# antbern/gridmap-slam-robot

Hardware: AMD Instinct MI355X
Metric: particle-scan evals/sec (higher is better)
Workload: dtype f64; 1 GPU; C3: 16384 particles/GPU x 720 beams (697 hits), 2048x2048 grid @ 0.02 m, full scan step (score+normalise+resample+ray-cast+likelihood rebuild; the rebuild is dirty-tile / factor-table-only: bit-identical results, likelihoodData on demand -- the reference's own every-cell rebuild is cpu_baseline.gpu_like_for_like_ms_per_step); particles_total=16384, particles_per_gpu=16384, beams=720, maps=1, maps_total=1, parallelism=single GPU, inputs=resident in HBM

## Files before the change

### gridmap_slam_robot_amd/csrc/gms_device.h

```cpp
#pragma once

#include <hip/hip_runtime.h>
#include <stdint.h>

#include "gms_internal.h"

#define GMS_WAVE 64

__device__ __forceinline__ void store_through(double *p, double v) { __hip_atomic_store(p, v, __ATOMIC_RELAXED, __HIP_MEMORY_SCOPE_AGENT); }
__device__ __forceinline__ void store_through(uint64_t *p, uint64_t v) { __hip_atomic_store(p, v, __ATOMIC_RELAXED, __HIP_MEMORY_SCOPE_AGENT); }

#define GMS_STAMP_SLOTS 16
#ifdef GMS_STAMPS
__device__ unsigned long long *g_gms_stamps;
#define GMS_STAMP_T(tid, row, slot) do { if (g_gms_stamps && threadIdx.x == (tid)) g_gms_stamps[(size_t)(row) * GMS_STAMP_SLOTS + (slot)] = wall_clock64(); } while (0)
#else
#define GMS_STAMP_T(tid, row, slot) do { } while (0)
#endif
#define GMS_STAMP(row, slot) GMS_STAMP_T(0, row, slot)
#define GMS_STAMP_ROW(kernel_id, wg) ((kernel_id) * 1024u + ((wg) < 1023u ? (wg) : 1023u))

__device__ __forceinline__ int32_t j_d2i(double d) {
    if (d != d) return 0;
    if (d >= 2147483647.0) return INT32_MAX;
    if (d <= -2147483648.0) return INT32_MIN;
// ... 200 lines not shown
```

### gridmap_slam_robot_amd/csrc/gms_fused_kernels.hip

```cpp
#include "gms_map_kernels.hip"
#include "gms_pf_kernels.hip"
#include "gms_slam_kernels.hip"

#ifndef GMS_APPLY_BLOCKS_RIDING
#define GMS_APPLY_BLOCKS_RIDING 512
#endif

#ifndef RCF_RAYS
#define RCF_RAYS 4
#endif

template <bool LOGNORM>
__global__ void __launch_bounds__(256)
k_norm_raycast(GridDev g, const gms_beam *__restrict__ beams, int32_t B, uint32_t *__restrict__ cnt, int32_t *__restrict__ bbox,
               int32_t nw_max, uint32_t n_ray_blocks,
               const double *__restrict__ partials, int64_t nblk_global, double *__restrict__ w, const float *__restrict__ pose,
               int32_t n, int64_t offset, PackedParticle *__restrict__ packed, double *__restrict__ cum,
               double *__restrict__ chunk_tot, int64_t nchunks, double *__restrict__ p2, PfStatsDev *__restrict__ stats,
               uint32_t n_norm_blocks, double *__restrict__ logd, uint32_t *__restrict__ cnt_pend, const int32_t *__restrict__ bbox_pend,
               uint32_t n_near_blocks, const double *__restrict__ logw_lognorm) {
    extern __shared__ __align__(16) unsigned char smem[];
    GMS_STAMP(GMS_STAMP_ROW(2, blockIdx.x), 0);
    if (blockIdx.x >= n_ray_blocks + n_norm_blocks) {
        apply_body(g, logd, cnt_pend, bbox_pend, nullptr, blockIdx.x - n_ray_blocks - n_norm_blocks, 0,
                   gridDim.x - n_ray_blocks - n_norm_blocks);
        GMS_STAMP(GMS_STAMP_ROW(2, blockIdx.x), 15);
        return;
    }
    if (blockIdx.x < n_ray_blocks) {
        __shared__ RedLds L;
        __shared__ float s_pose[3];
        const int cols[4] = { COL_SUM, COL_XW, COL_YW, COL_TW };
        double f[4];
        if (LOGNORM) {
            fold_lognorm<4>(partials, nblk_global, cols, f, L);
// ... 2 lines not shown
        }
        if (threadIdx.x == 0) {
            s_pose[0] = (float)(f[1] / f[0]);
            s_pose[1] = (float)(f[2] / f[0]);
            s_pose[2] = (float)(f[3] / f[0]);
        }
        __syncthreads();
        GMS_STAMP(GMS_STAMP_ROW(2, blockIdx.x), 1);
        if (blockIdx.x >= n_ray_blocks - n_near_blocks)
            raycast_near_body(g, beams, B, B, nullptr, 0, cnt, bbox, blockIdx.x - (n_ray_blocks - n_near_blocks), 0, smem, s_pose);
        else
            raycast_body<false, RCF_RAYS, 4>(g, beams, B, B, nullptr, 0, nullptr, cnt, bbox, nullptr, nullptr, 0, nullptr, nw_max, blockIdx.x, 0,
                                             smem, s_pose, n_near_blocks ? 1 : 0);
    } else {
        normalize_pack_body(partials, nblk_global, w, pose, n, offset, packed, cum, chunk_tot, nchunks, p2, stats,
                            blockIdx.x - n_ray_blocks, 0, LOGNORM ? logw_lognorm : (const double *)nullptr);
        GMS_STAMP(GMS_STAMP_ROW(2, blockIdx.x), 14);
    }
}

__global__ void __launch_bounds__(256)
k_partials_apply(double *__restrict__ w, double *__restrict__ logw, const float *__restrict__ pose, int32_t n, int64_t offset,
                 int64_t nblk_global, double *__restrict__ partials, const double *__restrict__ part, int32_t part_nseg,
                 GridDev g, double *__restrict__ logd, uint32_t *__restrict__ cnt, const int32_t *__restrict__ bbox,
                 int32_t *__restrict__ bbox_idle, PfStatsDev *__restrict__ lognorm_stats) {
    if (blockIdx.x < (uint32_t)nblk_global)
        partials_body(w, logw, pose, n, offset, nblk_global, partials, part, part_nseg, blockIdx.x, blockIdx.y, lognorm_stats);
    else
        apply_body(g, logd, cnt, bbox, bbox_idle, blockIdx.x - (uint32_t)nblk_global, blockIdx.y, gridDim.x - (uint32_t)nblk_global);
}

// ... 48 lines not shown
        chunk_sums_raw_body(glob_raw, n_global, nchunks, cum, chunk_tot, p2, nblk_global, partials,
                            blockIdx.x - n_ray_blocks - n_norm_blocks);
    }
}

template <int KH, int SPLIT>
__global__ void __launch_bounds__(256)
k_lik_resample(GridDev g, const double *__restrict__ logd, double *__restrict__ lik, double *__restrict__ fac, int64_t fac_stride,
               const double *__restrict__ taps_g, const int32_t *__restrict__ bbox, int32_t tiles_x, int32_t tiles_y,
               const uint32_t *__restrict__ cnt_pending, uint8_t *__restrict__ tile_state, uint32_t n_res_blocks,
               const PackedParticle *__restrict__ glob, int64_t n_global, int64_t nchunks, const double *__restrict__ cum,
               const double *__restrict__ chunk_off, const double *__restrict__ r01_maps, double r01, double fraction,
               int32_t n, int64_t offset,
               float *__restrict__ pose2, float *__restrict__ cs2, double *__restrict__ w2, int32_t *__restrict__ idx_out,
               const double *__restrict__ p2, int64_t nblk_global, PfStatsDev *__restrict__ stats, int32_t raw_weights,
               int32_t *__restrict__ bbox_clear, int32_t lik_mode) {
    extern __shared__ __align__(16) unsigned char smem[];
    GMS_STAMP(GMS_STAMP_ROW(3, blockIdx.x), 0);
    if (blockIdx.x == 0 && threadIdx.x < 4) bbox_clear[4 * blockIdx.y + threadIdx.x] = 0;
    if (blockIdx.x < n_res_blocks)
        resample_body(glob, n_global, nchunks, cum, chunk_off, r01_maps, r01, fraction, n, offset, pose2, cs2, w2, idx_out, p2,
                      nblk_global, stats, blockIdx.x, blockIdx.y, smem, raw_weights != 0);
    else
        likelihood_body<KH, SPLIT>(g, logd, lik, fac, fac_stride, taps_g, bbox, 1, tiles_x, tiles_y, blockIdx.x - n_res_blocks,
                                   blockIdx.y, gridDim.x - n_res_blocks, smem, cnt_pending, tile_state, lik_mode);
    GMS_STAMP(GMS_STAMP_ROW(3, blockIdx.x), blockIdx.x < n_res_blocks ? 1 : 2);
}

__global__ void __launch_bounds__(256)
k_deskew_motion(const double *__restrict__ angle, const double *__restrict__ distance, const uint8_t *__restrict__ hit, int32_t length,
                double d_center, double d_theta, gms_beam *__restrict__ beams_out, uint32_t n_deskew_blocks,
                float *__restrict__ pose, float *__restrict__ cs, int32_t n, int64_t offset, double d_center_sd, double d_theta_sd,
                uint64_t seed, uint64_t sequence) {
    if (blockIdx.x < n_deskew_blocks)
        deskew_body(angle, distance, hit, length, d_center, d_theta, beams_out, (int32_t)(blockIdx.x * 256u + threadIdx.x));
    else
        motion_body(pose, cs, n, offset, d_center, d_theta, d_center_sd, d_theta_sd, seed, sequence, 0,
                    (int32_t)((blockIdx.x - n_deskew_blocks) * 256u + threadIdx.x));
}

bool gms_can_pair_launches(const gms_pf *pf, int32_t B) {
    const gms_map *m = pf->map;
    return pf->n_maps == 1 && B > 0 && B <= GMS_MAX_BEAMS && !m->need_full_build && m->pair_launches;
}

void gms_launch_norm_raycast(gms_pf *pf, const double *d_partials, PackedParticle *d_packed_local, bool own,
                             const gms_beam *d_beams, int32_t B) {
    gms_map *m = pf->map;
    ProfScope ps(m, GMS_K_RAYCAST);
    if (own) { pf->d_global = pf->d_global_own; pf->global_raw = 0; }
    const uint32_t n_near = rc_near_blocks(m, B);
    const uint32_t n_ray = (uint32_t)((B + RCF_RAYS - 1) / RCF_RAYS) + n_near, n_norm = (uint32_t)((pf->n + 255) / 256);
    const size_t smem = rc_smem(m, RCF_RAYS, n_near);
    uint32_t n_apply = 0;
    if (m->apply_pending) {
        const int32_t all = ((m->gd.W + APPLY_TW - 1) / APPLY_TW) * ((m->gd.H + APPLY_TH - 1) / APPLY_TH);
        n_apply = (uint32_t)(all < GMS_APPLY_BLOCKS_RIDING ? all : GMS_APPLY_BLOCKS_RIDING);
    }
    int32_t *pend = m->d_bbox + (size_t)m->bbox_cur * 4;
    int32_t *bb = n_apply ? m->d_bbox + (size_t)(1 - m->bbox_cur) * 4 : pend;
    const bool lognorm = gms_pf_lognorm_now(pf);
#define NR_LAUNCH(LN)                                                                                                                 \
    do {                                                                                                                              \
        if (smem > 48 * 1024)                                                                                                         \
            hipFuncSetAttribute(reinterpret_cast<const void *>(&k_norm_raycast<LN>), hipFuncAttributeMaxDynamicSharedMemorySize, (int)smem); \
        hipLaunchKernelGGL(k_norm_raycast<LN>, dim3(n_ray + n_norm + n_apply), dim3(256), smem, m->stream, m->gd, d_beams, B, m->d_cnt, bb, \
                           rc_nw_max(m), n_ray, d_partials, nblk_global_of(pf), pf->d_w, pf->d_pose, pf->n, pf->offset, d_packed_local, \
                           own ? pf->d_cum : (double *)nullptr, own ? pf->d_chunk_tot : (double *)nullptr, nchunks_of(pf),          \
                           own ? pf->d_p2 : (double *)nullptr, pf->d_stats, n_norm, m->d_log, m->d_cnt_pend, pend, n_near,          \
                           LN ? (const double *)pf->d_logw : (const double *)nullptr);                                              \
    } while (0)
    if (lognorm) NR_LAUNCH(true); else NR_LAUNCH(false);
#undef NR_LAUNCH
    pf->score_fresh = 0;
    if (n_apply) gms_apply_done(m);
    pf->chunks_ready = own ? 1 : 0;
    pf->neff_folded = 0;
}

void gms_launch_partials_apply(gms_pf *pf, double *d_partials, bool apply_rides_later) {
    gms_map *m = pf->map;
    if (!m->apply_pending || apply_rides_later) { gms_launch_pf_partials(pf, d_partials); return; }
    ProfScope ps(m, GMS_K_REDUCE);
    const int64_t nblk = nblk_global_of(pf);
    const int32_t all = ((m->gd.W + APPLY_TW - 1) / APPLY_TW) * ((m->gd.H + APPLY_TH - 1) / APPLY_TH);
    const uint32_t n_apply = (uint32_t)(all < GMS_APPLY_BLOCKS ? all : GMS_APPLY_BLOCKS);
    int32_t *cur = m->d_bbox + (size_t)m->bbox_cur * m->n_maps * 4, *idle = m->d_bbox + (size_t)(1 - m->bbox_cur) * m->n_maps * 4;
    PfStatsDev *lognorm_stats = gms_pf_lognorm_now(pf) ? pf->d_stats : (PfStatsDev *)nullptr;
    hipLaunchKernelGGL(k_partials_apply, dim3((uint32_t)nblk + n_apply, pf->n_maps), dim3(256), 0, m->stream, pf->d_w, pf->d_logw,
                       pf->d_pose, pf->n, pf->offset, nblk, d_partials,
                       pf->pending_nseg ? (const double *)pf->d_part : (const double *)nullptr, pf->pending_nseg, m->gd, m->d_log,
                       m->d_cnt_pend, cur, idle, lognorm_stats);
    pf->pending_nseg = 0;
    gms_apply_done(m);
}

void gms_launch_lik_resample(gms_pf *pf, double fraction) {
    gms_map *m = pf->map;
    gms_launch_pf_chunk_sums(pf);
    ProfScope ps(m, GMS_K_LIKELIHOOD);
    const int32_t k = m->lik_kh;
    const int32_t tiles_x = (m->gd.W + LK_TW - 1) / LK_TW, tiles_y = (m->gd.H + LK_TH - 1) / LK_TH;
    const size_t smem_l = gms_likelihood_lds_bytes(m->gd.khalf, k != 0);
    int32_t blocks = tiles_x * tiles_y;
    const int32_t cap = gms_likelihood_blocks_cap(m, smem_l);
    if (blocks > cap) blocks = cap;
    blocks = (blocks + 7) & ~7;
    const int64_t nch = nchunks_of(pf);
    const size_t smem_r = gms_resample_lds_bytes(nch);
    const size_t smem = smem_l > smem_r ? smem_l : smem_r;
    const uint32_t n_res = (uint32_t)((pf->n + 255) / 256);
    const int32_t *bb = m->d_bbox + (size_t)m->bbox_cur * m->n_maps * 4;
    const double *r01_maps = pf->n_maps == 1 ? (const double *)nullptr : pf->d_r01_src;
    int32_t lik_mode = m->lik_lazy ? 2 : 3;
    if (m->lik_lazy) m->lik_stale = 1;
    if (m->fac_current && m->lik_skip) lik_mode |= 4;
    m->fac_current = 1;
    const bool split = k != 0 && gms_likelihood_split(m, blocks);
#define LR_LAUNCH(KH, SP)                                                                                                 \
    do {                                                                                                                  \
        if (smem > 48 * 1024)                                                                                             \
            hipFuncSetAttribute(reinterpret_cast<const void *>(&k_lik_resample<KH, SP>),                                 \
                                hipFuncAttributeMaxDynamicSharedMemorySize, (int)smem);                                   \
        hipLaunchKernelGGL((k_lik_resample<KH, SP>), dim3((uint32_t)blocks + n_res, pf->n_maps), dim3(256), smem, m->stream, m->gd, m->d_log, \
                           m->d_lik, m->d_fac, m->fac_stride, m->d_taps, bb, tiles_x, tiles_y, m->d_cnt, m->d_tile_state, n_res, pf->d_global, \
                           pf->n_global, nch, pf->d_cum, pf->d_chunk_tot, r01_maps, pf->r01_scalar, fraction, pf->n, pf->offset, \
                           pf->d_pose2, pf->d_cs2, pf->d_w2, pf->d_idx, pf->d_p2, nblk_global_of(pf), pf->d_stats,       \
                           pf->global_raw, m->d_bbox + (size_t)(1 - m->bbox_cur) * m->n_maps * 4, lik_mode);             \
    } while (0)
    if (k == 3) { if (split) LR_LAUNCH(3, 2); else LR_LAUNCH(3, 1); }
    else if (k == 5) { if (split) LR_LAUNCH(5, 2); else LR_LAUNCH(5, 1); }
    else LR_LAUNCH(0, 1);
#undef LR_LAUNCH
    pf->neff_folded = 1;
}

void gms_launch_partials_pack_apply(gms_pf *pf, bool apply_rides_later) {
    gms_map *m = pf->map;
    ProfScope ps(m, GMS_K_REDUCE);
    const uint32_t n_local = (uint32_t)((pf->n + GMS_BLOCK - 1) / GMS_BLOCK);
    uint32_t n_apply = 0;
    if (m->apply_pending && !apply_rides_later) {
        const int32_t all = ((m->gd.W + APPLY_TW - 1) / APPLY_TW) * ((m->gd.H + APPLY_TH - 1) / APPLY_TH);
// ... 23 lines not shown
        const int32_t all = ((m->gd.W + APPLY_TW - 1) / APPLY_TW) * ((m->gd.H + APPLY_TH - 1) / APPLY_TH);
        n_apply = (uint32_t)(all < GMS_APPLY_BLOCKS_RIDING ? all : GMS_APPLY_BLOCKS_RIDING);
    }
    int32_t *pend = m->d_bbox + (size_t)m->bbox_cur * 4;
    int32_t *bb = n_apply ? m->d_bbox + (size_t)(1 - m->bbox_cur) * 4 : pend;
    if (smem > 48 * 1024)
        hipFuncSetAttribute(reinterpret_cast<const void *>(&k_raycast_norm_chunks), hipFuncAttributeMaxDynamicSharedMemorySize,
                            (int)smem);
    hipLaunchKernelGGL(k_raycast_norm_chunks, dim3(n_ray + n_norm + n_chunk + n_apply), dim3(256), smem, m->stream, m->gd, d_beams, B,
                       m->d_cnt, bb, rc_nw_max(m), n_ray, n_norm, pf->d_partials, nblk_global_of(pf), pf->d_w, pf->d_pose, pf->n,
                       pf->offset, pf->d_global_own, pf->n_global, nchunks_of(pf), pf->d_cum, pf->d_chunk_tot, pf->d_p2, pf->d_stats,
                       n_chunk, m->d_log, m->d_cnt_pend, pend, n_near);
    if (n_apply) gms_apply_done(m);
    pf->chunks_ready = 1;
    pf->neff_folded = 0;
}

void gms_launch_deskew_motion(gms_pf *pf, const double *d_angle, const double *d_distance, const uint8_t *d_hit, int32_t length,
                              double d_center, double d_theta, uint64_t seed, uint64_t sequence) {
    gms_map *m = pf->map;
    const double d_center_sd = (0.01 + fabs(d_center) * 0.05) / 2;
    const double d_theta_sd = 5 * (3.141592653589793 / 180.0) + 0.1 * fabs(d_theta);
    const uint32_t n_dk = (uint32_t)((length + 255) / 256), n_mo = (uint32_t)((pf->n + 255) / 256);
    hipLaunchKernelGGL(k_deskew_motion, dim3(n_dk + n_mo), dim3(256), 0, m->stream, d_angle, d_distance, d_hit, length, d_center,
                       d_theta, m->d_beams, n_dk, pf->d_pose, pf->d_cs, pf->n, pf->offset, d_center_sd, d_theta_sd, seed, sequence);
}
```

### gridmap_slam_robot_amd/csrc/gms_host.hip

```cpp
#include <math.h>
#include <dlfcn.h>
#include <stdarg.h>
#include <stddef.h>
#include <stdio.h>
#include <stdlib.h>
#include <string.h>

#include <new>
#include <algorithm>
#include <vector>

#include "gms_internal.h"

static thread_local char g_err[512] = "";

static int fail(int code, const char *fmt, ...) {
    va_list ap;
    va_start(ap, fmt);
    vsnprintf(g_err, sizeof(g_err), fmt, ap);
    va_end(ap);
    return code;
}

int gms_fail(int code, const char *fmt, ...) {
// ... 798 lines not shown
    HIPCHK(hipMalloc(&d_a, n * sizeof(float)));
    HIPCHK(hipMalloc(&d_o, n * sizeof(float)));
    HIPCHK(hipMemcpyAsync(d_a, in, n * sizeof(float), hipMemcpyHostToDevice, m->stream));
    gms_launch_debug_f32(m, op, d_a, d_o, n);
    HIPCHK(hipMemcpyAsync(out, d_o, n * sizeof(float), hipMemcpyDeviceToHost, m->stream));
    HIPCHK(hipStreamSynchronize(m->stream));
    hipFree(d_a); hipFree(d_o);
    return GMS_OK;
}

static int64_t nblk_of(int64_t n) { return (n + GMS_BLOCK - 1) / GMS_BLOCK; }
static int64_t nchunks_of(int64_t n) { return (n + 63) / 64; }

static void pf_free_global(gms_pf *pf) {
    hipFree(pf->d_partials); hipFree(pf->d_p2); hipFree(pf->d_global_own); hipFree(pf->d_chunk_tot); hipFree(pf->d_cum);
    pf->d_partials = pf->d_p2 = nullptr; pf->d_global = pf->d_global_own = nullptr; pf->d_chunk_tot = pf->d_cum = nullptr;
}

static int pf_alloc_global(gms_pf *pf) {
    pf_free_global(pf);
    const size_t M = pf->n_maps;
    const size_t nblk = nblk_of(pf->n_global), nch = nchunks_of(pf->n_global);
    HIPCHK(hipMalloc(&pf->d_partials, M * nblk * GMS_PARTIAL_STRIDE * sizeof(double)));
    HIPCHK(hipMalloc(&pf->d_p2, M * nblk * 2 * sizeof(double)));
    HIPCHK(hipMalloc(&pf->d_global_own, M * pf->n_global * sizeof(PackedParticle)));
    pf->d_global = pf->d_global_own;
    HIPCHK(hipMalloc(&pf->d_chunk_tot, M * (nch + 1 + nch * 8) * sizeof(double)));
    HIPCHK(hipMalloc(&pf->d_cum, M * pf->n_global * sizeof(double)));
    return GMS_OK;
}

int gms_pf_destroy(gms_pf *pf) {
    if (!pf) return GMS_OK;
    hipSetDevice(pf->map->device);
    hipStreamSynchronize(pf->map->stream);
    pf->map->n_filters--;
    hipFree(pf->d_pose); hipFree(pf->d_pose2); hipFree(pf->d_part); hipFree(pf->d_cs2);
    hipFree(pf->d_w); hipFree(pf->d_w2); hipFree(pf->d_logw); hipFree(pf->d_cs); hipFree(pf->d_hitbeams);
    hipFree(pf->d_nhit); hipFree(pf->d_stats); hipFree(pf->d_r01); hipFree(pf->d_idx);
    hipFree(pf->d_ord); hipFree(pf->d_perm);
    pf_free_global(pf);
    if (pf->h_stats) hipHostFree(pf->h_stats);
    if (pf->h_stage) hipHostFree(pf->h_stage);
// ... 982 lines not shown
```

### gridmap_slam_robot_amd/csrc/gms_internal.h

```cpp
#pragma once

#include <hip/hip_runtime.h>
#include <stdint.h>

#include <vector>

#include "gridmapslam.h"

struct GridDev {
    int32_t W, H;
    int64_t cells;
    double posx, posy;
    double res;
    double rinv;
    float resf;
    double l_free, l_occ;
    int32_t extra;
    float half_tol;
    double z_hit;
    double c_rand;
    double inv_max;
    int32_t ktaps, khalf;
    int32_t fpitch;
    uint32_t fneutral;
// ... 119 lines not shown
    float *d_cs2;
    double *d_w, *d_w2;
    double *d_logw, *d_logw2;
    float *d_cs;
    double *d_hitbeams;
    double *d_part;
    int32_t *d_nhit;
    double *d_partials;
    double *d_p2;
    int32_t neff_folded;
    int32_t global_raw;
    PackedParticle *d_global_own;
    PackedParticle *d_global;
    double *d_chunk_tot;
    double *d_cum;
    PfStatsDev *d_stats;
    int32_t stats_current;
    PfStatsDev *h_stats;
    double *d_r01;
    const double *d_r01_src;
    double r01_scalar;
    int32_t *d_idx;
    float *h_stage;
    StageRing pose_ring;
    StageRing r01_ring;
    int32_t have_global;
    int32_t chunks_ready;
    int32_t refine;
    int32_t pending_nseg;
    float4 *d_ord;
// ... 141 lines not shown
```

### gridmap_slam_robot_amd/csrc/gms_pf_kernels.hip

```cpp
#include "gms_device.h"

#define SCAN_CHUNK 64
#define RES_SUB_MAX_CHUNKS 1024

__global__ void k_pf_init(float *pose, float *cs, double *w, double *logw, int64_t total, double w0) {
    int64_t i = (int64_t)blockIdx.x * blockDim.x + threadIdx.x;
    if (i < total) {
        pose[3 * i] = 0.0f; pose[3 * i + 1] = 0.0f; pose[3 * i + 2] = 0.0f;
        cs[2 * i] = 1.0f; cs[2 * i + 1] = 0.0f;
        w[i] = w0; logw[i] = 0.0;
    }
}

__global__ void __launch_bounds__(256)
k_pose_trig(const float *__restrict__ src, float *__restrict__ dst, float *__restrict__ cs, int64_t total) {
    const int64_t i = (int64_t)blockIdx.x * blockDim.x + threadIdx.x;
    if (i >= total) return;
    const float x = src[3 * i], y = src[3 * i + 1], th = src[3 * i + 2];
    dst[3 * i] = x; dst[3 * i + 1] = y; dst[3 * i + 2] = th;
    float c, s;
    pose_trig(th, c, s);
    cs[2 * i] = c; cs[2 * i + 1] = s;
}

// ... 625 lines not shown
        if (glob) {
            const PackedParticle pp = glob[s->strongest];
            s->spose[0] = pp.x; s->spose[1] = pp.y; s->spose[2] = pp.theta;
        } else if (pose && st >= 0 && st < pose_n) {
            s->spose[0] = pose[3 * st]; s->spose[1] = pose[3 * st + 1]; s->spose[2] = pose[3 * st + 2];
        }
    }
    return sum;
}

__device__ __forceinline__ int64_t block_count(int64_t n, int64_t blk) {
    const int64_t left = n - blk * GMS_BLOCK;
    return left < 0 ? 0 : (left > GMS_BLOCK ? GMS_BLOCK : left);
}

__device__ __forceinline__ void fold_neff(const double *__restrict__ p2, int64_t nblk, double &norm_sum, double &sq_sum,
                                          double *lds) {
    double a = 0.0, q = 0.0;
    for (int64_t b = threadIdx.x & (GRP - 1); b < nblk; b += GRP) { a += p2[2 * b]; q += p2[2 * b + 1]; }
    norm_sum = group_sum(a, lds);
    const double qq = group_sum(q, lds);
    sq_sum = qq / (norm_sum * norm_sum);
}

__global__ void __launch_bounds__(256)
k_fold_neff(const double *__restrict__ p2_all, int64_t nblk, PfStatsDev *__restrict__ stats) {
    __shared__ RedLds L;
    const int32_t mi = blockIdx.x;
    double ns, sq;
    fold_neff(p2_all + (size_t)mi * nblk * 2, nblk, ns, sq, L.a);
    if (threadIdx.x == 0) { stats[mi].norm_sum = ns; stats[mi].sq_sum = sq; }
}

__device__ __forceinline__ void
// ... 21 lines not shown

__global__ void __launch_bounds__(256)
k_partials(double *__restrict__ w, double *__restrict__ logw, const float *__restrict__ pose, int32_t n,
           int64_t offset, int64_t nblk_global, double *__restrict__ partials, const double *__restrict__ part,
           int32_t part_nseg, PfStatsDev *__restrict__ lognorm_stats) {
    GMS_STAMP(GMS_STAMP_ROW(1, blockIdx.x), 0);
    partials_body(w, logw, pose, n, offset, nblk_global, partials, part, part_nseg, blockIdx.x, blockIdx.y, lognorm_stats);
    GMS_STAMP(GMS_STAMP_ROW(1, blockIdx.x), 1);
}

__device__ __forceinline__ double *chunk_sub_of(double *chunk_tot_all, int64_t nchunks, int32_t n_maps, int32_t mi) {
    return chunk_tot_all + (size_t)n_maps * (nchunks + 1) + (size_t)mi * nchunks * 8;
}
__device__ __forceinline__ void block_chunk_scan(double v, int64_t i, int64_t n_pop, int64_t blk, int64_t nchunks,
                                                 double *__restrict__ cum, double *__restrict__ chunk_tot,
                                                 double *__restrict__ p2_blk, double *__restrict__ sub) {
    __shared__ double s_ct[4][2];
    const int32_t lane = threadIdx.x & 63, wave = threadIdx.x >> 6;
    double inc = v;
#pragma unroll
    for (int o = 1; o < 64; o <<= 1) {
        const double up = __shfl_up(inc, o, GMS_WAVE);
        if (lane >= o) inc += up;
    }
    const double sq = wave_sum_f64(v * v);
    const double tot = __shfl(inc, 63, GMS_WAVE);
    if (i < n_pop) cum[i] = inc;
    if ((lane & 7) == 7 && blk * 4 + wave < nchunks) sub[(blk * 4 + wave) * 8 + (lane >> 3)] = inc;
    if (lane == 0) {
        const int64_t c = blk * 4 + wave;
        if (c < nchunks) chunk_tot[c] = tot;
        s_ct[wave][0] = tot; s_ct[wave][1] = sq;
    }
    __syncthreads();
    if (threadIdx.x == 0) {
        p2_blk[0] = ((s_ct[0][0] + s_ct[1][0]) + s_ct[2][0]) + s_ct[3][0];
        p2_blk[1] = ((s_ct[0][1] + s_ct[1][1]) + s_ct[2][1]) + s_ct[3][1];
    }
}
static_assert(4 * SCAN_CHUNK == GMS_BLOCK, "a reduction block is four scan chunks");

__device__ __forceinline__ void
normalize_pack_body(const double *__restrict__ partials_all, int64_t nblk_global, double *__restrict__ w,
                    const float *__restrict__ pose, int32_t n, int64_t offset, PackedParticle *__restrict__ packed,
                    double *__restrict__ cum, double *__restrict__ chunk_tot, int64_t nchunks,
                    double *__restrict__ p2_all, PfStatsDev *__restrict__ stats, uint32_t bx, uint32_t by,
                    const double *__restrict__ logw_lognorm = nullptr) {
    __shared__ RedLds L;
    const int32_t mi = (int32_t)by;
    const double *p = partials_all + (size_t)mi * nblk_global * GMS_PARTIAL_STRIDE;
    double M = 0.0;
    const double sum = fold_stats(p, nblk_global, stats + mi, bx == 0, pose + (size_t)mi * n * 3, offset, n, L, nullptr, logw_lognorm != nullptr, &M);
    const int32_t i = (int32_t)bx * 256 + threadIdx.x;
    double wn = 0.0;
    if (logw_lognorm) {
        const double v = i < n ? exp(logw_lognorm[(size_t)mi * n + i] - lognorm_ref(M)) : 1.0;
        const int32_t zeros = __popcll(__ballot(v == 0.0));
        if ((threadIdx.x & 63) == 0 && zeros) atomicAdd(&stats[mi].n_zero, zeros);
        if (i < n) w[(size_t)mi * n + i] = v;
    }
    if (i < n) {
        const size_t gi = (size_t)mi * n + i;
        wn = w[gi] / sum;
        w[gi] = wn;
        PackedParticle pp;
        pp.w = wn; pp.x = pose[3 * gi]; pp.y = pose[3 * gi + 1]; pp.theta = pose[3 * gi + 2]; pp.pad = 0u;
        packed[gi] = pp;
    }
    if (cum)
        block_chunk_scan(wn, i, n, bx, nchunks, cum + (size_t)mi * n, chunk_tot + (size_t)mi * (nchunks + 1),
                         p2_all + ((size_t)mi * nblk_global + bx) * 2, chunk_sub_of(chunk_tot, nchunks, (int32_t)gridDim.y, mi));
}

__global__ void __launch_bounds__(256)
k_normalize_pack(const double *__restrict__ partials_all, int64_t nblk_global, double *__restrict__ w,
                 const float *__restrict__ pose, int32_t n, int64_t offset, PackedParticle *__restrict__ packed,
                 double *__restrict__ cum, double *__restrict__ chunk_tot, int64_t nchunks,
                 double *__restrict__ p2_all, PfStatsDev *__restrict__ stats, const double *__restrict__ logw_lognorm) {
    normalize_pack_body(partials_all, nblk_global, w, pose, n, offset, packed, cum, chunk_tot, nchunks, p2_all, stats, blockIdx.x,
                        blockIdx.y, logw_lognorm);
}

__device__ __forceinline__ void
chunk_sums_body(const PackedParticle *__restrict__ glob_all, int64_t n_global, int64_t nchunks, double *__restrict__ cum_all,
                double *__restrict__ chunk_tot, double *__restrict__ p2_all, int64_t nblk_global, PfStatsDev *__restrict__ stats,
                uint32_t bx, uint32_t by) {
// ... 63 lines not shown
                       PackedParticle *__restrict__ packed) {
    const int32_t mi = blockIdx.y;
    const int32_t i = blockIdx.x * blockDim.x + threadIdx.x;
    if (i >= n) return;
    const size_t gi = (size_t)mi * n + i;
    PackedParticle pp;
    pp.w = w[gi]; pp.x = pose[3 * gi]; pp.y = pose[3 * gi + 1]; pp.theta = pose[3 * gi + 2]; pp.pad = 0u;
    packed[gi] = pp;
}

__device__ __forceinline__ void
resample_body(const PackedParticle *__restrict__ glob_all, int64_t n_global, int64_t nchunks,
              const double *__restrict__ cum_all, const double *__restrict__ chunk_off, const double *__restrict__ r01,
              double r01_scalar, double fraction, int32_t n, int64_t offset, float *__restrict__ pose2, float *__restrict__ cs2,
              double *__restrict__ w2, int32_t *__restrict__ idx_out, const double *__restrict__ p2_all, int64_t nblk_global,
              PfStatsDev *__restrict__ stats, uint32_t bx, uint32_t by, unsigned char *smem, bool raw_weights = false) {
    double *off = reinterpret_cast<double *>(smem);
    const int32_t mi = (int32_t)by;
    __shared__ RedLds L;
    const double *tot = chunk_off + (size_t)mi * (nchunks + 1);
    double tv[8];
#pragma unroll
    for (int k = 0; k < 8; k++) { const int64_t c = (int64_t)threadIdx.x + k * (int64_t)blockDim.x; tv[k] = c < nchunks ? tot[c] : 0.0; }
    const bool use_sub = nchunks <= RES_SUB_MAX_CHUNKS;
    double *sub = reinterpret_cast<double *>(smem) + (nchunks + 1) + ((nchunks + 63) / 64 + 1);
    const double *sub_g = chunk_sub_of(const_cast<double *>(chunk_off), nchunks, (int32_t)gridDim.y, mi);
    if (use_sub) {
        for (int64_t e0 = (int64_t)threadIdx.x; e0 < nchunks * 8; e0 += 8 * (int64_t)blockDim.x) {
            double v[8];
#pragma unroll
            for (int k = 0; k < 8; k++) { const int64_t e = e0 + k * (int64_t)blockDim.x; v[k] = e < nchunks * 8 ? sub_g[e] : 0.0; }
#pragma unroll
            for (int k = 0; k < 8; k++) { const int64_t e = e0 + k * (int64_t)blockDim.x; if (e < nchunks * 8) sub[e] = v[k]; }
        }
    }
    double norm_sum, sq_sum;
    fold_neff(p2_all + (size_t)mi * nblk_global * 2, nblk_global, norm_sum, sq_sum, L.a);
    if (bx == 0 && threadIdx.x == 0) { stats[mi].norm_sum = norm_sum; stats[mi].sq_sum = sq_sum; }
    GMS_STAMP(GMS_STAMP_ROW(3, blockIdx.x), 5);
    const bool go = fraction < 0.0 || (1.0 / sq_sum) < fraction * (double)n_global;
    const int64_t nsuper = (nchunks + 63) / 64;
    double *sup = off + nchunks + 1;
    if (go) {
#pragma unroll
        for (int k = 0; k < 8; k++) { const int64_t c = (int64_t)threadIdx.x + k * (int64_t)blockDim.x; if (c < nchunks) off[c] = tv[k]; }
        for (int64_t c0 = (int64_t)threadIdx.x + 8 * (int64_t)blockDim.x; c0 < nchunks; c0 += 8 * (int64_t)blockDim.x) {
            double v[8];
#pragma unroll
            for (int k = 0; k < 8; k++) { const int64_t c = c0 + k * (int64_t)blockDim.x; v[k] = c < nchunks ? tot[c] : 0.0; }
#pragma unroll
            for (int k = 0; k < 8; k++) { const int64_t c = c0 + k * (int64_t)blockDim.x; if (c < nchunks) off[c] = v[k]; }
        }
        __syncthreads();
        for (int64_t sidx = threadIdx.x >> 6; sidx < nsuper; sidx += blockDim.x >> 6) {
            const int32_t lane = threadIdx.x & 63;
            const int64_t c = sidx * 64 + lane;
            const double v = c < nchunks ? off[c] : 0.0;
            double inc = v;
#pragma unroll
            for (int o = 1; o < 64; o <<= 1) {
                const double up = __shfl_up(inc, o, GMS_WAVE);
                if (lane >= o) inc += up;
            }
            const double excl = __shfl_up(inc, 1, GMS_WAVE);
            if (c < nchunks) off[c] = lane == 0 ? 0.0 : excl;
            if (lane == 63) sup[sidx] = inc;
        }
        __syncthreads();
        if (threadIdx.x < 64) {
            const int32_t lane = threadIdx.x;
            double carry = 0.0;
            for (int64_t s0 = 0; s0 < nsuper; s0 += 64) {
                const int64_t sidx = s0 + lane;
                const double v = sidx < nsuper ? sup[sidx] : 0.0;
                double inc = v;
#pragma unroll
                for (int o = 1; o < 64; o <<= 1) {
                    const double up = __shfl_up(inc, o, GMS_WAVE);
                    if (lane >= o) inc += up;
                }
                const double excl = __shfl_up(inc, 1, GMS_WAVE);
                if (sidx < nsuper) sup[sidx] = s0 == 0 ? (lane == 0 ? 0.0 : excl) : carry + (lane == 0 ? 0.0 : excl);
                const double tot = __shfl(inc, 63, GMS_WAVE);
                carry = s0 == 0 ? tot : carry + tot;
            }
            if (lane == 0) off[nchunks] = carry;
        }
        __syncthreads();
        for (int64_t c = 64 + threadIdx.x; c < nchunks; c += blockDim.x) off[c] = sup[c >> 6] + off[c];
        __syncthreads();
    }
    GMS_STAMP(GMS_STAMP_ROW(3, blockIdx.x), 6);
    const int32_t t = (int32_t)bx * blockDim.x + threadIdx.x;
    if (t >= n) return;
    const PackedParticle *g = glob_all + (size_t)mi * n_global;
    const int64_t m0 = offset + t;
    int64_t src = m0;
    if (go) {
        const double *cm = cum_all + (size_t)mi * n_global;
        const double N = (double)n_global;
        const double r = (r01 ? r01[mi] : r01_scalar) * 1.0 / N;
        const double U = r + (double)m0 * 1.0 / N;
        int64_t lo = 0, hi = nchunks;
        while (lo < hi) {
            const int64_t mid = (lo + hi) >> 1;
// ... 410 lines not shown
    pf->pending_nseg = 0;
}

void gms_launch_pf_apply_partials(gms_pf *pf, const double *d_partials, PackedParticle *d_packed_local, bool own) {
    gms_map *m = pf->map;
    ProfScope ps(m, GMS_K_REDUCE);
    const int64_t nblk = nblk_global_of(pf);
    if (own) { pf->d_global = pf->d_global_own; pf->global_raw = 0; }
    hipLaunchKernelGGL(k_normalize_pack, dim3((pf->n + 255) / 256, pf->n_maps), dim3(256), 0, m->stream, d_partials, nblk,
                       pf->d_w, pf->d_pose, pf->n, pf->offset, d_packed_local, own ? pf->d_cum : (double *)nullptr,
                       own ? pf->d_chunk_tot : (double *)nullptr, nchunks_of(pf), own ? pf->d_p2 : (double *)nullptr, pf->d_stats,
                       gms_pf_lognorm_now(pf) ? (const double *)pf->d_logw : (const double *)nullptr);
    pf->score_fresh = 0;
    pf->chunks_ready = own ? 1 : 0;
    pf->neff_folded = 0;
}

void gms_launch_pf_stats_only(gms_pf *pf, const double *d_partials, PfStatsDev *d_stats_out) {
    gms_map *m = pf->map;
    ProfScope ps(m, GMS_K_REDUCE);
    hipLaunchKernelGGL(k_stats_only, dim3(pf->n_maps), dim3(256), 0, m->stream, d_partials, nblk_global_of(pf), pf->d_pose,
                       pf->n, pf->offset, d_stats_out);
}

void gms_launch_pf_pack(gms_pf *pf, PackedParticle *d_packed) {
    gms_map *m = pf->map;
    hipLaunchKernelGGL(k_pack, dim3((pf->n + 255) / 256, pf->n_maps), dim3(256), 0, m->stream, pf->d_w, pf->d_pose,
                       pf->n, d_packed);
    if (d_packed == pf->d_global) { pf->chunks_ready = 0; pf->neff_folded = 0; pf->global_raw = 0; }
}

void gms_launch_pf_chunk_sums(gms_pf *pf) {
    if (pf->chunks_ready) return;
    gms_map *m = pf->map;
    ProfScope ps(m, GMS_K_RESAMPLE);
    const int64_t nch = nchunks_of(pf);
    hipLaunchKernelGGL(k_chunk_sums, dim3((unsigned)nblk_global_of(pf), pf->n_maps), dim3(256), 0, m->stream, pf->d_global,
                       pf->n_global, nch, pf->d_cum, pf->d_chunk_tot, pf->d_p2, nblk_global_of(pf), pf->d_stats);
    pf->chunks_ready = 1;
}

void gms_launch_pf_fold_neff(gms_pf *pf) {
    if (pf->neff_folded) return;
    gms_map *m = pf->map;
    gms_launch_pf_chunk_sums(pf);
    hipLaunchKernelGGL(k_fold_neff, dim3(pf->n_maps), dim3(256), 0, m->stream, pf->d_p2, nblk_global_of(pf), pf->d_stats);
    pf->neff_folded = 1;
}

void gms_launch_pf_after_gather(gms_pf *pf) {
    pf->global_raw = 0;
    pf->chunks_ready = 0;
    pf->neff_folded = 0;
    gms_launch_pf_chunk_sums(pf);
}

void gms_launch_pf_resample(gms_pf *pf, double fraction) {
    gms_map *m = pf->map;
    gms_launch_pf_chunk_sums(pf);
    ProfScope ps(m, GMS_K_RESAMPLE);
    const int64_t nch = nchunks_of(pf);
    const size_t smem = gms_resample_lds_bytes(nch);
    if (smem > 48 * 1024)
        hipFuncSetAttribute(reinterpret_cast<const void *>(&k_resample), hipFuncAttributeMaxDynamicSharedMemorySize,
                            (int)smem);
    hipLaunchKernelGGL(k_resample, dim3((pf->n + 255) / 256, pf->n_maps), dim3(256), smem, m->stream, pf->d_global,
                       pf->n_global, nch, pf->d_cum, pf->d_chunk_tot, pf->n_maps == 1 ? (const double *)nullptr : pf->d_r01_src,
                       pf->r01_scalar, fraction, pf->n, pf->offset,
// ... 30 lines not shown
```

Before: 365.6 million particle-scan evals/s.

## Precompute resample chunk-offset prefix in last normalize block via atomic ticket

The normalize-pack blocks now write chunk totals and per-block weight sums with write-through stores and take an atomic ticket. The last block to arrive folds the effective-sample-size sums, scans the chunk offsets, and stores the prefix plus norms in a new buffer. The resample blocks in the following likelihood/resample kernel then load this precomputed prefix instead of each redoing the fold and chunk-offset scan. The cost is a serial tail in the raycast kernel, where a single block does the scan, plus extra host state flags that must be invalidated correctly.

```diff
diff --git a/gridmap_slam_robot_amd/csrc/gms_device.h b/gridmap_slam_robot_amd/csrc/gms_device.h
--- a/gridmap_slam_robot_amd/csrc/gms_device.h
+++ b/gridmap_slam_robot_amd/csrc/gms_device.h
@@ -9,6 +9,10 @@
 
 __device__ __forceinline__ void store_through(double *p, double v) { __hip_atomic_store(p, v, __ATOMIC_RELAXED, __HIP_MEMORY_SCOPE_AGENT); }
 __device__ __forceinline__ void store_through(uint64_t *p, uint64_t v) { __hip_atomic_store(p, v, __ATOMIC_RELAXED, __HIP_MEMORY_SCOPE_AGENT); }
+template <bool COHERENT>
+__device__ __forceinline__ double load_coherent(const double *p) {
+    return COHERENT ? __hip_atomic_load(p, __ATOMIC_RELAXED, __HIP_MEMORY_SCOPE_AGENT) : *p;
+}
 
 #define GMS_STAMP_SLOTS 16
 #ifdef GMS_STAMPS
diff --git a/gridmap_slam_robot_amd/csrc/gms_fused_kernels.hip b/gridmap_slam_robot_amd/csrc/gms_fused_kernels.hip
--- a/gridmap_slam_robot_amd/csrc/gms_fused_kernels.hip
+++ b/gridmap_slam_robot_amd/csrc/gms_fused_kernels.hip
@@ -18,7 +18,8 @@
                int32_t n, int64_t offset, PackedParticle *__restrict__ packed, double *__restrict__ cum,
                double *__restrict__ chunk_tot, int64_t nchunks, double *__restrict__ p2, PfStatsDev *__restrict__ stats,
                uint32_t n_norm_blocks, double *__restrict__ logd, uint32_t *__restrict__ cnt_pend, const int32_t *__restrict__ bbox_pend,
-               uint32_t n_near_blocks, const double *__restrict__ logw_lognorm) {
+               uint32_t n_near_blocks, const double *__restrict__ logw_lognorm, uint32_t *__restrict__ res_ticket,
+               double *__restrict__ res_pre) {
     extern __shared__ __align__(16) unsigned char smem[];
     GMS_STAMP(GMS_STAMP_ROW(2, blockIdx.x), 0);
     if (blockIdx.x >= n_ray_blocks + n_norm_blocks) {
@@ -51,7 +52,8 @@
                                              smem, s_pose, n_near_blocks ? 1 : 0);
     } else {
         normalize_pack_body(partials, nblk_global, w, pose, n, offset, packed, cum, chunk_tot, nchunks, p2, stats,
-                            blockIdx.x - n_ray_blocks, 0, LOGNORM ? logw_lognorm : (const double *)nullptr);
+                            blockIdx.x - n_ray_blocks, 0, LOGNORM ? logw_lognorm : (const double *)nullptr, res_ticket, n_norm_blocks,
+                            res_pre, smem);
         GMS_STAMP(GMS_STAMP_ROW(2, blockIdx.x), 14);
     }
 }
@@ -130,13 +132,13 @@
                int32_t n, int64_t offset,
                float *__restrict__ pose2, float *__restrict__ cs2, double *__restrict__ w2, int32_t *__restrict__ idx_out,
                const double *__restrict__ p2, int64_t nblk_global, PfStatsDev *__restrict__ stats, int32_t raw_weights,
-               int32_t *__restrict__ bbox_clear, int32_t lik_mode) {
+               int32_t *__restrict__ bbox_clear, int32_t lik_mode, const double *__restrict__ res_pre) {
     extern __shared__ __align__(16) unsigned char smem[];
     GMS_STAMP(GMS_STAMP_ROW(3, blockIdx.x), 0);
     if (blockIdx.x == 0 && threadIdx.x < 4) bbox_clear[4 * blockIdx.y + threadIdx.x] = 0;
     if (blockIdx.x < n_res_blocks)
         resample_body(glob, n_global, nchunks, cum, chunk_off, r01_maps, r01, fraction, n, offset, pose2, cs2, w2, idx_out, p2,
-                      nblk_global, stats, blockIdx.x, blockIdx.y, smem, raw_weights != 0);
+                      nblk_global, stats, blockIdx.x, blockIdx.y, smem, raw_weights != 0, res_pre);
     else
         likelihood_body<KH, SPLIT>(g, logd, lik, fac, fac_stride, taps_g, bbox, 1, tiles_x, tiles_y, blockIdx.x - n_res_blocks,
                                    blockIdx.y, gridDim.x - n_res_blocks, smem, cnt_pending, tile_state, lik_mode);
@@ -167,7 +169,10 @@
     if (own) { pf->d_global = pf->d_global_own; pf->global_raw = 0; }
     const uint32_t n_near = rc_near_blocks(m, B);
     const uint32_t n_ray = (uint32_t)((B + RCF_RAYS - 1) / RCF_RAYS) + n_near, n_norm = (uint32_t)((pf->n + 255) / 256);
-    const size_t smem = rc_smem(m, RCF_RAYS, n_near);
+    const int64_t nch = nchunks_of(pf);
+    const size_t smem_pre = own ? (size_t)(nch + 1 + (nch + 63) / 64 + 1) * sizeof(double) : 0;
+    size_t smem = rc_smem(m, RCF_RAYS, n_near);
+    if (smem < smem_pre) smem = smem_pre;
     uint32_t n_apply = 0;
     if (m->apply_pending) {
         const int32_t all = ((m->gd.W + APPLY_TW - 1) / APPLY_TW) * ((m->gd.H + APPLY_TH - 1) / APPLY_TH);
@@ -184,14 +189,16 @@
                            rc_nw_max(m), n_ray, d_partials, nblk_global_of(pf), pf->d_w, pf->d_pose, pf->n, pf->offset, d_packed_local, \
                            own ? pf->d_cum : (double *)nullptr, own ? pf->d_chunk_tot : (double *)nullptr, nchunks_of(pf),          \
                            own ? pf->d_p2 : (double *)nullptr, pf->d_stats, n_norm, m->d_log, m->d_cnt_pend, pend, n_near,          \
-                           LN ? (const double *)pf->d_logw : (const double *)nullptr);                                              \
+                           LN ? (const double *)pf->d_logw : (const double *)nullptr, own ? pf->d_res_ticket : (uint32_t *)nullptr,       \
+                           pf->d_res_pre);                                                                                              \
     } while (0)
     if (lognorm) NR_LAUNCH(true); else NR_LAUNCH(false);
 #undef NR_LAUNCH
     pf->score_fresh = 0;
     if (n_apply) gms_apply_done(m);
     pf->chunks_ready = own ? 1 : 0;
-    pf->neff_folded = 0;
+    pf->neff_folded = own ? 1 : 0;
+    pf->res_pre_ready = own ? 1 : 0;
 }
 
 void gms_launch_partials_apply(gms_pf *pf, double *d_partials, bool apply_rides_later) {
@@ -214,6 +221,8 @@
 void gms_launch_lik_resample(gms_pf *pf, double fraction) {
     gms_map *m = pf->map;
     gms_launch_pf_chunk_sums(pf);
+    const double *pre = pf->res_pre_ready ? (const double *)pf->d_res_pre : (const double *)nullptr;
+    pf->res_pre_ready = 0;
     ProfScope ps(m, GMS_K_LIKELIHOOD);
     const int32_t k = m->lik_kh;
     const int32_t tiles_x = (m->gd.W + LK_TW - 1) / LK_TW, tiles_y = (m->gd.H + LK_TH - 1) / LK_TH;
@@ -242,7 +251,7 @@
                            m->d_lik, m->d_fac, m->fac_stride, m->d_taps, bb, tiles_x, tiles_y, m->d_cnt, m->d_tile_state, n_res, pf->d_global, \
                            pf->n_global, nch, pf->d_cum, pf->d_chunk_tot, r01_maps, pf->r01_scalar, fraction, pf->n, pf->offset, \
                            pf->d_pose2, pf->d_cs2, pf->d_w2, pf->d_idx, pf->d_p2, nblk_global_of(pf), pf->d_stats,       \
-                           pf->global_raw, m->d_bbox + (size_t)(1 - m->bbox_cur) * m->n_maps * 4, lik_mode);             \
+                           pf->global_raw, m->d_bbox + (size_t)(1 - m->bbox_cur) * m->n_maps * 4, lik_mode, pre);        \
     } while (0)
     if (k == 3) { if (split) LR_LAUNCH(3, 2); else LR_LAUNCH(3, 1); }
     else if (k == 5) { if (split) LR_LAUNCH(5, 2); else LR_LAUNCH(5, 1); }
@@ -296,6 +305,7 @@
     if (n_apply) gms_apply_done(m);
     pf->chunks_ready = 1;
     pf->neff_folded = 0;
+    pf->res_pre_ready = 0;
 }
 
 void gms_launch_deskew_motion(gms_pf *pf, const double *d_angle, const double *d_distance, const uint8_t *d_hit, int32_t length,
diff --git a/gridmap_slam_robot_amd/csrc/gms_host.hip b/gridmap_slam_robot_amd/csrc/gms_host.hip
--- a/gridmap_slam_robot_amd/csrc/gms_host.hip
+++ b/gridmap_slam_robot_amd/csrc/gms_host.hip
@@ -836,7 +836,9 @@
 
 static void pf_free_global(gms_pf *pf) {
     hipFree(pf->d_partials); hipFree(pf->d_p2); hipFree(pf->d_global_own); hipFree(pf->d_chunk_tot); hipFree(pf->d_cum);
+    hipFree(pf->d_res_pre); hipFree(pf->d_res_ticket);
     pf->d_partials = pf->d_p2 = nullptr; pf->d_global = pf->d_global_own = nullptr; pf->d_chunk_tot = pf->d_cum = nullptr;
+    pf->d_res_pre = nullptr; pf->d_res_ticket = nullptr; pf->res_pre_ready = 0;
 }
 
 static int pf_alloc_global(gms_pf *pf) {
@@ -849,6 +851,9 @@
     pf->d_global = pf->d_global_own;
     HIPCHK(hipMalloc(&pf->d_chunk_tot, M * (nch + 1 + nch * 8) * sizeof(double)));
     HIPCHK(hipMalloc(&pf->d_cum, M * pf->n_global * sizeof(double)));
+    HIPCHK(hipMalloc(&pf->d_res_pre, M * (nch + 3) * sizeof(double)));
+    HIPCHK(hipMalloc(&pf->d_res_ticket, M * sizeof(uint32_t)));
+    HIPCHK(hipMemsetAsync(pf->d_res_ticket, 0, M * sizeof(uint32_t), pf->map->stream));
     return GMS_OK;
 }
 
diff --git a/gridmap_slam_robot_amd/csrc/gms_internal.h b/gridmap_slam_robot_amd/csrc/gms_internal.h
--- a/gridmap_slam_robot_amd/csrc/gms_internal.h
+++ b/gridmap_slam_robot_amd/csrc/gms_internal.h
@@ -157,6 +157,9 @@
     PackedParticle *d_global;
     double *d_chunk_tot;
     double *d_cum;
+    double *d_res_pre;
+    uint32_t *d_res_ticket;
+    int32_t res_pre_ready;
     PfStatsDev *d_stats;
     int32_t stats_current;
     PfStatsDev *h_stats;
diff --git a/gridmap_slam_robot_amd/csrc/gms_pf_kernels.hip b/gridmap_slam_robot_amd/csrc/gms_pf_kernels.hip
--- a/gridmap_slam_robot_amd/csrc/gms_pf_kernels.hip
+++ b/gridmap_slam_robot_amd/csrc/gms_pf_kernels.hip
@@ -663,10 +663,11 @@
     return left < 0 ? 0 : (left > GMS_BLOCK ? GMS_BLOCK : left);
 }
 
+template <bool COHERENT = false>
 __device__ __forceinline__ void fold_neff(const double *__restrict__ p2, int64_t nblk, double &norm_sum, double &sq_sum,
                                           double *lds) {
     double a = 0.0, q = 0.0;
-    for (int64_t b = threadIdx.x & (GRP - 1); b < nblk; b += GRP) { a += p2[2 * b]; q += p2[2 * b + 1]; }
+    for (int64_t b = threadIdx.x & (GRP - 1); b < nblk; b += GRP) { a += load_coherent<COHERENT>(&p2[2 * b]); q += load_coherent<COHERENT>(&p2[2 * b + 1]); }
     norm_sum = group_sum(a, lds);
     const double qq = group_sum(q, lds);
     sq_sum = qq / (norm_sum * norm_sum);
@@ -718,7 +719,7 @@
 }
 __device__ __forceinline__ void block_chunk_scan(double v, int64_t i, int64_t n_pop, int64_t blk, int64_t nchunks,
                                                  double *__restrict__ cum, double *__restrict__ chunk_tot,
-                                                 double *__restrict__ p2_blk, double *__restrict__ sub) {
+                                                 double *__restrict__ p2_blk, double *__restrict__ sub, bool through = false) {
     __shared__ double s_ct[4][2];
     const int32_t lane = threadIdx.x & 63, wave = threadIdx.x >> 6;
     double inc = v;
@@ -733,23 +734,105 @@
     if ((lane & 7) == 7 && blk * 4 + wave < nchunks) sub[(blk * 4 + wave) * 8 + (lane >> 3)] = inc;
     if (lane == 0) {
         const int64_t c = blk * 4 + wave;
-        if (c < nchunks) chunk_tot[c] = tot;
+        if (c < nchunks) { if (through) store_through(&chunk_tot[c], tot); else chunk_tot[c] = tot; }
         s_ct[wave][0] = tot; s_ct[wave][1] = sq;
     }
     __syncthreads();
     if (threadIdx.x == 0) {
-        p2_blk[0] = ((s_ct[0][0] + s_ct[1][0]) + s_ct[2][0]) + s_ct[3][0];
-        p2_blk[1] = ((s_ct[0][1] + s_ct[1][1]) + s_ct[2][1]) + s_ct[3][1];
+        const double a = ((s_ct[0][0] + s_ct[1][0]) + s_ct[2][0]) + s_ct[3][0];
+        const double q = ((s_ct[0][1] + s_ct[1][1]) + s_ct[2][1]) + s_ct[3][1];
+        if (through) { store_through(&p2_blk[0], a); store_through(&p2_blk[1], q); } else { p2_blk[0] = a; p2_blk[1] = q; }
     }
 }
 static_assert(4 * SCAN_CHUNK == GMS_BLOCK, "a reduction block is four scan chunks");
+
+__device__ __forceinline__ void chunk_offsets_scan(double *off, int64_t nchunks) {
+    const int64_t nsuper = (nchunks + 63) / 64;
+    double *sup = off + nchunks + 1;
+    __syncthreads();
+    for (int64_t sidx = threadIdx.x >> 6; sidx < nsuper; sidx += blockDim.x >> 6) {
+        const int32_t lane = threadIdx.x & 63;
+        const int64_t c = sidx * 64 + lane;
+        const double v = c < nchunks ? off[c] : 0.0;
+        double inc = v;
+#pragma unroll
+        for (int o = 1; o < 64; o <<= 1) {
+            const double up = __shfl_up(inc, o, GMS_WAVE);
+            if (lane >= o) inc += up;
+        }
+        const double excl = __shfl_up(inc, 1, GMS_WAVE);
+        if (c < nchunks) off[c] = lane == 0 ? 0.0 : excl;
+        if (lane == 63) sup[sidx] = inc;
+    }
+    __syncthreads();
+    if (threadIdx.x < 64) {
+        const int32_t lane = threadIdx.x;
+        double carry = 0.0;
+        for (int64_t s0 = 0; s0 < nsuper; s0 += 64) {
+            const int64_t sidx = s0 + lane;
+            const double v = sidx < nsuper ? sup[sidx] : 0.0;
+            double inc = v;
+#pragma unroll
+            for (int o = 1; o < 64; o <<= 1) {
+                const double up = __shfl_up(inc, o, GMS_WAVE);
+                if (lane >= o) inc += up;
+            }
+            const double excl = __shfl_up(inc, 1, GMS_WAVE);
+            if (sidx < nsuper) sup[sidx] = s0 == 0 ? (lane == 0 ? 0.0 : excl) : carry + (lane == 0 ? 0.0 : excl);
+            const double tot = __shfl(inc, 63, GMS_WAVE);
+            carry = s0 == 0 ? tot : carry + tot;
+        }
+        if (lane == 0) off[nchunks] = carry;
+    }
+    __syncthreads();
+    for (int64_t c = 64 + threadIdx.x; c < nchunks; c += blockDim.x) off[c] = sup[c >> 6] + off[c];
+    __syncthreads();
+}
+
+__device__ __forceinline__ void
+resample_prefix_last(const double *__restrict__ p2, int64_t nblk, const double *__restrict__ tot, int64_t nchunks, uint32_t *__restrict__ ticket,
+                     uint32_t n_blocks, double *__restrict__ pre, PfStatsDev *__restrict__ stats, unsigned char *smem, double *lds) {
+    __shared__ int32_t s_last;
+    asm volatile("s_waitcnt vmcnt(0)" ::: "memory");
+    __syncthreads();
+    if (threadIdx.x == 0) {
+        const uint32_t t = __hip_atomic_fetch_add(ticket, 1u, __ATOMIC_RELAXED, __HIP_MEMORY_SCOPE_AGENT);
+        s_last = t == n_blocks - 1;
+        if (s_last) __hip_atomic_store(ticket, 0u, __ATOMIC_RELAXED, __HIP_MEMORY_SCOPE_AGENT);
+    }
+    __syncthreads();
+    if (!s_last) return;
+    double *off = reinterpret_cast<double *>(smem);
+    double tv[8];
+#pragma unroll
+    for (int k = 0; k < 8; k++) { const int64_t c = (int64_t)threadIdx.x + k * (int64_t)blockDim.x; tv[k] = c < nchunks ? load_coherent<true>(&tot[c]) : 0.0; }
+    double norm_sum, sq_sum;
+    fold_neff<true>(p2, nblk, norm_sum, sq_sum, lds);
+#pragma unroll
+    for (int k = 0; k < 8; k++) { const int64_t c = (int64_t)threadIdx.x + k * (int64_t)blockDim.x; if (c < nchunks) off[c] = tv[k]; }
+    for (int64_t c0 = (int64_t)threadIdx.x + 8 * (int64_t)blockDim.x; c0 < nchunks; c0 += 8 * (int64_t)blockDim.x) {
+        double v[8];
+#pragma unroll
+        for (int k = 0; k < 8; k++) { const int64_t c = c0 + k * (int64_t)blockDim.x; v[k] = c < nchunks ? load_coherent<true>(&tot[c]) : 0.0; }
+#pragma unroll
+        for (int k = 0; k < 8; k++) { const int64_t c = c0 + k * (int64_t)blockDim.x; if (c < nchunks) off[c] = v[k]; }
+    }
+    chunk_offsets_scan(off, nchunks);
+    for (int64_t c = threadIdx.x; c <= nchunks; c += blockDim.x) pre[c] = off[c];
+    if (threadIdx.x == 0) {
+        pre[nchunks + 1] = norm_sum; pre[nchunks + 2] = sq_sum;
+        stats->norm_sum = norm_sum; stats->sq_sum = sq_sum;
+    }
+    GMS_STAMP(GMS_STAMP_ROW(2, blockIdx.x), 13);
+}
 
 __device__ __forceinline__ void
 normalize_pack_body(const double *__restrict__ partials_all, int64_t nblk_global, double *__restrict__ w,
                     const float *__restrict__ pose, int32_t n, int64_t offset, PackedParticle *__restrict__ packed,
                     double *__restrict__ cum, double *__restrict__ chunk_tot, int64_t nchunks,
                     double *__restrict__ p2_all, PfStatsDev *__restrict__ stats, uint32_t bx, uint32_t by,
-                    const double *__restrict__ logw_lognorm = nullptr) {
+                    const double *__restrict__ logw_lognorm = nullptr, uint32_t *__restrict__ ticket = nullptr,
+                    uint32_t n_blocks = 0, double *__restrict__ pre = nullptr, unsigned char *smem = nullptr) {
     __shared__ RedLds L;
     const int32_t mi = (int32_t)by;
     const double *p = partials_all + (size_t)mi * nblk_global * GMS_PARTIAL_STRIDE;
@@ -773,7 +856,10 @@
     }
     if (cum)
         block_chunk_scan(wn, i, n, bx, nchunks, cum + (size_t)mi * n, chunk_tot + (size_t)mi * (nchunks + 1),
-                         p2_all + ((size_t)mi * nblk_global + bx) * 2, chunk_sub_of(chunk_tot, nchunks, (int32_t)gridDim.y, mi));
+                         p2_all + ((size_t)mi * nblk_global + bx) * 2, chunk_sub_of(chunk_tot, nchunks, (int32_t)gridDim.y, mi),
+                         ticket != nullptr);
+    if (cum && ticket) resample_prefix_last(p2_all + (size_t)mi * nblk_global * 2, nblk_global, chunk_tot + (size_t)mi * (nchunks + 1),
+                                            nchunks, ticket + mi, n_blocks, pre + (size_t)mi * (nchunks + 3), stats + mi, smem, L.a);
 }
 
 __global__ void __launch_bounds__(256)
@@ -867,14 +953,16 @@
               const double *__restrict__ cum_all, const double *__restrict__ chunk_off, const double *__restrict__ r01,
               double r01_scalar, double fraction, int32_t n, int64_t offset, float *__restrict__ pose2, float *__restrict__ cs2,
               double *__restrict__ w2, int32_t *__restrict__ idx_out, const double *__restrict__ p2_all, int64_t nblk_global,
-              PfStatsDev *__restrict__ stats, uint32_t bx, uint32_t by, unsigned char *smem, bool raw_weights = false) {
+              PfStatsDev *__restrict__ stats, uint32_t bx, uint32_t by, unsigned char *smem, bool raw_weights = false,
+              const double *__restrict__ pre = nullptr) {
     double *off = reinterpret_cast<double *>(smem);
     const int32_t mi = (int32_t)by;
     __shared__ RedLds L;
-    const double *tot = chunk_off + (size_t)mi * (nchunks + 1);
+    const double *tot = pre ? pre + (size_t)mi * (nchunks + 3) : chunk_off + (size_t)mi * (nchunks + 1);
+    const int64_t nload = pre ? nchunks + 1 : nchunks;
     double tv[8];
 #pragma unroll
-    for (int k = 0; k < 8; k++) { const int64_t c = (int64_t)threadIdx.x + k * (int64_t)blockDim.x; tv[k] = c < nchunks ? tot[c] : 0.0; }
+    for (int k = 0; k < 8; k++) { const int64_t c = (int64_t)threadIdx.x + k * (int64_t)blockDim.x; tv[k] = c < nload ? tot[c] : 0.0; }
     const bool use_sub = nchunks <= RES_SUB_MAX_CHUNKS;
     double *sub = reinterpret_cast<double *>(smem) + (nchunks + 1) + ((nchunks + 63) / 64 + 1);
     const double *sub_g = chunk_sub_of(const_cast<double *>(chunk_off), nchunks, (int32_t)gridDim.y, mi);
@@ -888,60 +976,26 @@
         }
     }
     double norm_sum, sq_sum;
-    fold_neff(p2_all + (size_t)mi * nblk_global * 2, nblk_global, norm_sum, sq_sum, L.a);
-    if (bx == 0 && threadIdx.x == 0) { stats[mi].norm_sum = norm_sum; stats[mi].sq_sum = sq_sum; }
+    if (pre) {
+        sq_sum = tot[nchunks + 2];
+    } else {
+        fold_neff(p2_all + (size_t)mi * nblk_global * 2, nblk_global, norm_sum, sq_sum, L.a);
+        if (bx == 0 && threadIdx.x == 0) { stats[mi].norm_sum = norm_sum; stats[mi].sq_sum = sq_sum; }
+    }
     GMS_STAMP(GMS_STAMP_ROW(3, blockIdx.x), 5);
     const bool go = fraction < 0.0 || (1.0 / sq_sum) < fraction * (double)n_global;
-    const int64_t nsuper = (nchunks + 63) / 64;
-    double *sup = off + nchunks + 1;
     if (go) {
 #pragma unroll
-        for (int k = 0; k < 8; k++) { const int64_t c = (int64_t)threadIdx.x + k * (int64_t)blockDim.x; if (c < nchunks) off[c] = tv[k]; }
-        for (int64_t c0 = (int64_t)threadIdx.x + 8 * (int64_t)blockDim.x; c0 < nchunks; c0 += 8 * (int64_t)blockDim.x) {
+        for (int k = 0; k < 8; k++) { const int64_t c = (int64_t)threadIdx.x + k * (int64_t)blockDim.x; if (c < nload) off[c] = tv[k]; }
+        for (int64_t c0 = (int64_t)threadIdx.x + 8 * (int64_t)blockDim.x; c0 < nload; c0 += 8 * (int64_t)blockDim.x) {
             double v[8];
 #pragma unroll
-            for (int k = 0; k < 8; k++) { const int64_t c = c0 + k * (int64_t)blockDim.x; v[k] = c < nchunks ? tot[c] : 0.0; }
-#pragma unroll
-            for (int k = 0; k < 8; k++) { const int64_t c = c0 + k * (int64_t)blockDim.x; if (c < nchunks) off[c] = v[k]; }
-        }
-        __syncthreads();
-        for (int64_t sidx = threadIdx.x >> 6; sidx < nsuper; sidx += blockDim.x >> 6) {
-            const int32_t lane = threadIdx.x & 63;
-            const int64_t c = sidx * 64 + lane;
-            const double v = c < nchunks ? off[c] : 0.0;
-            double inc = v;
-#pragma unroll
-            for (int o = 1; o < 64; o <<= 1) {
-                const double up = __shfl_up(inc, o, GMS_WAVE);
-                if (lane >= o) inc += up;
-            }
-            const double excl = __shfl_up(inc, 1, GMS_WAVE);
-            if (c < nchunks) off[c] = lane == 0 ? 0.0 : excl;
-            if (lane == 63) sup[sidx] = inc;
-        }
-        __syncthreads();
-        if (threadIdx.x < 64) {
-            const int32_t lane = threadIdx.x;
-            double carry = 0.0;
-            for (int64_t s0 = 0; s0 < nsuper; s0 += 64) {
-                const int64_t sidx = s0 + lane;
-                const double v = sidx < nsuper ? sup[sidx] : 0.0;
-                double inc = v;
-#pragma unroll
-                for (int o = 1; o < 64; o <<= 1) {
-                    const double up = __shfl_up(inc, o, GMS_WAVE);
-                    if (lane >= o) inc += up;
-                }
-                const double excl = __shfl_up(inc, 1, GMS_WAVE);
-                if (sidx < nsuper) sup[sidx] = s0 == 0 ? (lane == 0 ? 0.0 : excl) : carry + (lane == 0 ? 0.0 : excl);
-                const double tot = __shfl(inc, 63, GMS_WAVE);
-                carry = s0 == 0 ? tot : carry + tot;
-            }
-            if (lane == 0) off[nchunks] = carry;
-        }
-        __syncthreads();
-        for (int64_t c = 64 + threadIdx.x; c < nchunks; c += blockDim.x) off[c] = sup[c >> 6] + off[c];
-        __syncthreads();
+            for (int k = 0; k < 8; k++) { const int64_t c = c0 + k * (int64_t)blockDim.x; v[k] = c < nload ? tot[c] : 0.0; }
+#pragma unroll
+            for (int k = 0; k < 8; k++) { const int64_t c = c0 + k * (int64_t)blockDim.x; if (c < nload) off[c] = v[k]; }
+        }
+        if (pre) __syncthreads();
+        else chunk_offsets_scan(off, nchunks);
     }
     GMS_STAMP(GMS_STAMP_ROW(3, blockIdx.x), 6);
     const int32_t t = (int32_t)bx * blockDim.x + threadIdx.x;
@@ -1382,6 +1436,7 @@
     pf->score_fresh = 0;
     pf->chunks_ready = own ? 1 : 0;
     pf->neff_folded = 0;
+    pf->res_pre_ready = 0;
 }
 
 void gms_launch_pf_stats_only(gms_pf *pf, const double *d_partials, PfStatsDev *d_stats_out) {
@@ -1395,7 +1450,7 @@
     gms_map *m = pf->map;
     hipLaunchKernelGGL(k_pack, dim3((pf->n + 255) / 256, pf->n_maps), dim3(256), 0, m->stream, pf->d_w, pf->d_pose,
                        pf->n, d_packed);
-    if (d_packed == pf->d_global) { pf->chunks_ready = 0; pf->neff_folded = 0; pf->global_raw = 0; }
+    if (d_packed == pf->d_global) { pf->chunks_ready = 0; pf->neff_folded = 0; pf->global_raw = 0; pf->res_pre_ready = 0; }
 }
 
 void gms_launch_pf_chunk_sums(gms_pf *pf) {
@@ -1406,6 +1461,7 @@
     hipLaunchKernelGGL(k_chunk_sums, dim3((unsigned)nblk_global_of(pf), pf->n_maps), dim3(256), 0, m->stream, pf->d_global,
                        pf->n_global, nch, pf->d_cum, pf->d_chunk_tot, pf->d_p2, nblk_global_of(pf), pf->d_stats);
     pf->chunks_ready = 1;
+    pf->res_pre_ready = 0;
 }
 
 void gms_launch_pf_fold_neff(gms_pf *pf) {
@@ -1420,6 +1476,7 @@
     pf->global_raw = 0;
     pf->chunks_ready = 0;
     pf->neff_folded = 0;
+    pf->res_pre_ready = 0;
     gms_launch_pf_chunk_sums(pf);
 }
 
```

Result: faster. 373.3 million particle-scan evals/s (median of 6 runs) (+2.1%).
